# JuanJoZP/cfd-hemodynamic

Measured on AMD Instinct MI355X. Metric: time-steps/sec, dfg_1 ~1M DOF (stabilized_schur), higher is better.
Workload: dtype f64 (fp32 only in the AMG matrix values of the flexible preconditioner and in a read-only copy of the Krylov basis that Gram-Schmidt reads in solves of >= 20 iterations)

## Files before the change

cfd_hemodynamic_amd/_lib.py:

```python
from __future__ import annotations

import ctypes as C
import os
import subprocess

import numpy as np

_HERE = os.path.dirname(os.path.abspath(__file__))
_SO = os.path.join(_HERE, "libcfdh.so")
_LIB = None

dp = C.POINTER(C.c_double)
ip = C.POINTER(C.c_int32)
lp = C.POINTER(C.c_int64)


class Options(C.Structure):
    _fields_ = [
        ("snes_rtol", C.c_double), ("snes_atol", C.c_double), ("snes_stol", C.c_double), ("snes_max_it", C.c_int32),
        ("ksp_rtol", C.c_double), ("ksp_atol", C.c_double), ("ksp_max_it", C.c_int32), ("ksp_restart", C.c_int32),
        ("cheb_degree", C.c_int32), ("cheb_ratio", C.c_double), ("schur_full", C.c_int32),
        ("amg_smooth_degree", C.c_int32), ("amg_smooth_ratio", C.c_double), ("amg_theta", C.c_double),
        ("amg_max_coarse", C.c_int32), ("pc_refresh", C.c_int32), ("remove_p_mean", C.c_int32), ("verbose", C.c_int32),
        ("pc_type", C.c_int32), ("cc_smooth_degree", C.c_int32), ("ksp_guess", C.c_int32),
# ... 14 lines not shown
        ("ms_solve", C.c_double * 3), ("ms_total", C.c_double), ("launches", C.c_int32), ("host_syncs", C.c_int32),
    ]


ALLREDUCE_FN = C.CFUNCTYPE(C.c_int, C.c_void_p, dp, C.c_int, C.c_int)
EXCHANGE_FN = C.CFUNCTYPE(C.c_int, C.c_void_p, dp, dp)

SYMBOLS = [
    "cfdh_create", "cfdh_create_elem", "cfdh_create_elem_part", "cfdh_set_facet_markers", "cfdh_destroy", "cfdh_last_error", "cfdh_abi_version", "cfdh_set_params", "cfdh_default_options",
    "cfdh_set_options", "cfdh_clear_dirichlet", "cfdh_add_dirichlet", "cfdh_update_dirichlet", "cfdh_set_state", "cfdh_get_solution",
    "cfdh_get_previous", "cfdh_get_residual", "cfdh_advance", "cfdh_advance_field", "cfdh_set_time_scheme", "cfdh_set_previous2", "cfdh_get_previous2",
    "cfdh_shift_history", "cfdh_set_boundary_terms", "cfdh_set_formulation", "cfdh_set_pressure_boundaries", "cfdh_set_pressure_boundaries_ex", "cfdh_assemble", "cfdh_get_csr", "cfdh_spmv", "cfdh_solve_step",
    "cfdh_functional", "cfdh_wall_shear_stress", "cfdh_set_global_pressure_space", "cfdh_set_halo", "cfdh_comm_unique_id", "cfdh_comm_init", "cfdh_comm_set_callbacks",
    "cfdh_profile_enable", "cfdh_profile_get", "cfdh_profile_reset", "cfdh_info",
    "cfdh_set_schur_pcd", "cfdh_set_ksp_forcing", "cfdh_get_newton_history", "cfdh_get_pcd_operator", "cfdh_apply_preconditioner", "cfdh_apply_operator",
    "cfdh_get_amg_operator", "cfdh_get_amg_vectors", "cfdh_krylov_vec_op",
    "cfdh_create_ipcs", "cfdh_ipcs_set_form", "cfdh_ipcs_set_tolerances", "cfdh_ipcs_step", "cfdh_ipcs_get_operator", "cfdh_ipcs_get_intermediate",
    "cfdh_ipcs_apply_pressure_pc", "cfdh_ipcs_krylov_solve",
    "cfdh_wall_stats_reset", "cfdh_wall_stats_accumulate", "cfdh_wall_stats_get",
]


def build(force=False):
    src = os.path.join(_HERE, "csrc")
    newest = max(os.path.getmtime(os.path.join(src, f)) for f in os.listdir(src)
                 if f.endswith((".hip", ".cpp", ".hpp", ".h")))
    hdr = os.path.join(os.path.dirname(_HERE), "include", "cfdh.h")
    if os.path.exists(hdr):
        newest = max(newest, os.path.getmtime(hdr))
    if force or not os.path.exists(_SO) or os.path.getmtime(_SO) < newest:
# ... 51 lines not shown
    L.cfdh_set_global_pressure_space.argtypes = [vp, C.c_int64, C.c_int64, ip, dp, ip, C.c_int64, ip]
    L.cfdh_comm_unique_id.argtypes = [C.c_void_p]
    L.cfdh_comm_init.argtypes = [vp, C.c_void_p, C.c_int, C.c_int]
    L.cfdh_comm_set_callbacks.argtypes = [vp, ALLREDUCE_FN, EXCHANGE_FN, C.c_void_p, C.c_int, C.c_int]
    L.cfdh_profile_enable.argtypes = [vp, C.c_int]
    L.cfdh_profile_get.argtypes = [vp, C.c_int, dp, lp]
    L.cfdh_profile_reset.argtypes = [vp]
    L.cfdh_info.argtypes = [vp, C.c_int]
    L.cfdh_info.restype = C.c_int64
    L.cfdh_set_schur_pcd.argtypes = [vp, C.c_int, C.c_int, C.c_int]
    L.cfdh_set_ksp_forcing.argtypes = [vp, C.c_int, C.c_double, C.c_double, C.c_double, C.c_double, C.c_double]
    L.cfdh_get_newton_history.argtypes = [vp, ip, dp, dp, ip, dp]
    L.cfdh_get_pcd_operator.argtypes = [vp, lp, ip, ip, dp, dp]
    L.cfdh_apply_preconditioner.argtypes = [vp, dp, dp]
    L.cfdh_apply_operator.argtypes = [vp, dp, dp, dp]
    L.cfdh_get_amg_operator.argtypes = [vp, C.c_int, C.c_int, C.c_int, lp, lp, lp, ip, ip, dp]
    L.cfdh_get_amg_vectors.argtypes = [vp, C.c_int, C.c_int, C.c_int, lp, dp]
    L.cfdh_krylov_vec_op.argtypes = [vp, C.c_int, C.c_int, C.c_int, C.c_int, dp, dp, dp, dp, dp, C.c_double, C.c_int, dp, dp,
                                     C.POINTER(C.c_float), ip, dp, dp, dp]
    L.cfdh_create_ipcs.argtypes = [C.POINTER(vp), C.c_int, C.c_int, C.c_int64, C.c_int64, C.c_int64, ip, dp, C.c_int64, ip, ip, ip]
    L.cfdh_ipcs_set_form.argtypes = [vp, C.c_double, C.c_double]
    L.cfdh_ipcs_set_tolerances.argtypes = [vp, dp, C.c_double, ip]
    L.cfdh_ipcs_step.argtypes = [vp, C.POINTER(IpcsStats)]
    L.cfdh_ipcs_get_operator.argtypes = [vp, C.c_int, lp, ip, ip, dp]
    L.cfdh_ipcs_get_intermediate.argtypes = [vp, C.c_int, dp]
    L.cfdh_ipcs_apply_pressure_pc.argtypes = [vp, dp, dp]
    L.cfdh_ipcs_krylov_solve.argtypes = [vp, C.c_int, dp, dp, C.c_double, C.c_double, C.c_int, dp, C.POINTER(IpcsStats), dp]
    L.cfdh_wall_stats_reset.argtypes = [vp]
    L.cfdh_wall_stats_accumulate.argtypes = [vp, C.c_double]
    L.cfdh_wall_stats_get.argtypes = [vp, C.c_int, lp, dp]
# ... 318 lines not shown
        if r.size != (self.dim + 1) * self.nv:
            raise ValueError("monolithic vector of (gdim + 1) nv entries expected")
        z = np.zeros_like(r)
        self._chk(self.L.cfdh_apply_preconditioner(self.h, _dp(r), _dp(z)))
        return z

    def apply_operator(self, r):
        r = np.ascontiguousarray(r, dtype=np.float64)
        if r.size != (self.dim + 1) * self.nv:
            raise ValueError("monolithic vector of (gdim + 1) nv entries expected")
        z = np.zeros_like(r)
        w = np.zeros((self.dim + 1) * self.nvo)
        self._chk(self.L.cfdh_apply_operator(self.h, _dp(r), _dp(z), _dp(w)))
        return z, w

    def krylov_vec_op(self, op, n, ld, nvec=1, A=None, B=None, x=None, y=None, coef=None, scalar=0.0, flags=0):
        def arr(a, need, what):
            if a is None:
                return None
            a = np.ascontiguousarray(a, dtype=np.float64).ravel()
            if a.size < need:
                raise ValueError("%s: %d entries, %d needed" % (what, a.size, need))
            return a
        blk = max(n, 0) if op == KVOP_NORM2_TRIPLE else max(ld, 0) * max(nvec, 0)
        ncoef = {KVOP_GS_UPDATE_NORMALIZE: nvec + 1, KVOP_GUESS: 8 * (nvec + 1)}.get(op, nvec)
        A, B = arr(A, blk, "A"), arr(B, blk, "B")
        x, y, coef = arr(x, n, "x"), arr(y, n, "y"), arr(coef, ncoef, "coef")
        m = max(n, 1)
        out1, out2, out32 = np.zeros(m), np.zeros(m), np.zeros(m, dtype=np.float32)
        ns = max(nvec + 2, 72)
# ... 145 lines not shown
```

cfd_hemodynamic_amd/csrc/cfdh_api.cpp:

```cpp
#include <algorithm>
#include <cmath>
#include <numeric>

#include <dlfcn.h>

#include "cfdh_internal.hpp"
#include "cfdh_ipcs.hpp"

std::string g_cfdh_last_error;

int cfdh_prepare_assembly(cfdh_ctx *c);

#define ENTER(c)                         \
  do {                                   \
    if (!(c)) return CFDH_E_ARG;         \
    (void)hipSetDevice((c)->device);     \
  } while (0)

#define NOT_IPCS(c, name)                                                                                                    \
  do {                                                                                                                       \
    if ((c) && (c)->ipcs) return cfdh_fail((c), CFDH_E_STATE, name ": not available on an incremental pressure-correction context (cfdh_create_ipcs)"); \
  } while (0)
#define NEED_IPCS(c, name)                                                                                         \
  do {                                                                                                             \
// ... 63 lines not shown
  *out = nullptr;
  if (gdim != 2 && gdim != 3) return cfdh_fail(nullptr, CFDH_E_ARG, "gdim must be 2 (P1 triangles) or 3 (P1 tetrahedra)");
  if (etype < 0 || etype > 3) return cfdh_fail(nullptr, CFDH_E_ARG, "unknown element type %d", etype);
  if (!cells || !coords || (nfacets > 0 && (!facet_cells || !facet_local)))
    return cfdh_fail(nullptr, CFDH_E_ARG, "null mesh array");
  int ndev = 0;
  if (hipGetDeviceCount(&ndev) != hipSuccess || ndev <= 0)
    return cfdh_fail(nullptr, CFDH_E_HIP, "no HIP device available: libcfdh has no CPU fallback");
  if (device < 0 || device >= ndev) return cfdh_fail(nullptr, CFDH_E_ARG, "device %d out of range (%d devices)", device, ndev);
  cfdh_ctx *c = new (std::nothrow) cfdh_ctx();
  if (!c) return cfdh_fail(nullptr, CFDH_E_NOMEM, "out of host memory");
  c->device = device;
  cfdh_default_options(&c->opt);
  { const char *e = getenv("CFDH_NO_GRAPH"); c->use_graph = !(e && e[0] == '1'); }
  { const char *e = getenv("CFDH_SOLVE_LEAN"); c->lean = !(e && e[0] == '0'); }
  {
    cfdh_ctx::SolveEnv &v = c->env;
    const char *e;
    if ((e = getenv("CFDH_KRYLOV_FP32"))) v.krylov_fp32 = atoi(e);
    v.guess_check = getenv("CFDH_GUESS_CHECK") != nullptr;
    e = getenv("CFDH_NO_ATTAINABLE_STOP"); v.no_attainable_stop = e && e[0] == '1';
    if ((e = getenv("CFDH_GS_REFINE_FROM"))) v.gs_refine_from = atoi(e);
    if ((e = getenv("CFDH_KSP_LAG"))) v.ksp_lag = atoi(e);
    if ((e = getenv("CFDH_GS_ETA2"))) v.gs_eta2 = atof(e);
    if ((e = getenv("CFDH_L_CYCLES"))) v.l_cycles = atoi(e);
    if ((e = getenv("CFDH_A_CYCLES"))) v.a_cycles = atoi(e);
    e = getenv("CFDH_DL0_COARSE_SWEEPS"); v.dl0_coarse_sweeps = e && e[0] == '1';
  }
  if (c->use_graph && (getenv("ROCP_TOOL_LIBRARIES") || dlsym(RTLD_DEFAULT, "rocprofiler_configure"))) {
    int rt = 0;
// ... 550 lines not shown

int cfdh_apply_operator(cfdh_ctx *c, const double *r, double *z, double *w) {
  NOT_IPCS(c, "cfdh_apply_operator");
  if (!c || !r || !z || !w) return CFDH_E_ARG;
  ENTER(c);
  if (c->nranks > 1 || c->nvo != c->nv) return cfdh_fail(c, CFDH_E_STATE, "cfdh_apply_operator: one GPU only");
  if (!c->jac_valid) return cfdh_fail(c, CFDH_E_STATE, "no Jacobian assembled yet");
  CHK(cfdh_pc_update(c, false));
  std::vector<double> h;
  pack_vec(c, r, r + (size_t)c->dim * c->nv, h, nullptr);
  CHK(upload_vec(c, h, c->xt.p));
  CHK(cfdh_apply_operator_dev(c, c->xt.p, c->dvec.p));
  std::vector<double> oz, ow;
  CHK(download_vec(c, c->dvec.p, oz));
  CHK(download_vec(c, c->kw.p, ow));
  for (int k = 0; k < c->nvo; k++) {
    const int v = c->iperm[k], d = c->dim;
    for (int i = 0; i < d; i++) { z[(size_t)d * v + i] = oz[(size_t)d * k + i]; w[(size_t)d * v + i] = ow[(size_t)d * k + i]; }
    z[(size_t)d * c->nv + v] = oz[(size_t)d * c->nvo + k];
    w[(size_t)d * c->nvo + v] = ow[(size_t)d * c->nvo + k];
  }
  return 0;
}

int cfdh_krylov_vec_op(cfdh_ctx *c, int op, int n, int ld, int nvec, const double *A, const double *B, const double *x, const double *y,
                       const double *coef, double scalar, int flags, double *out1, double *out2, float *out32, int32_t *nscal,
                       double *scal_host, double *scal_dev, double *scal_mirror) {
  NOT_IPCS(c, "cfdh_krylov_vec_op");
  ENTER(c);
  if (c->nranks > 1 || c->nvo != c->nv) return cfdh_fail(c, CFDH_E_STATE, "cfdh_krylov_vec_op: one GPU only");
// ... 716 lines not shown
int cfdh_profile_get(cfdh_ctx *c, int kind, double *total_ms, int64_t *launches) {
  NOT_IPCS(c, "cfdh_profile_get");
  if (!c || kind < 0 || kind >= 12) return CFDH_E_ARG;
  prof_flush(c);
  if (total_ms) *total_ms = c->prof[kind].total_ms;
  if (launches) *launches = c->prof[kind].launches;
  return 0;
}
int cfdh_profile_reset(cfdh_ctx *c) {
  NOT_IPCS(c, "cfdh_profile_reset");
  ENTER(c);
  prof_flush(c);
  for (auto &p : c->prof) { p.total_ms = 0; p.launches = 0; }
  c->n_allreduce = c->n_halo = c->n_host_sync = c->n_krylov = c->n_allgather = 0;
  c->n_cycles = c->n_guess_projections = c->n_iter_sync = 0;
  c->n_krylov_discarded = 0;
  return 0;
}

int64_t cfdh_info(const cfdh_ctx *c, int what) {
  if (!c) return -1;
  if (c->ipcs) {
    const IpcsData *I = c->ipcs;
    switch (what) {
      case 0: case 1: return I->nn;
      case 2: return I->nc;
      case 3: return (int64_t)I->hM.col.size();
      case 6: return (int64_t)I->hLam.lev.size();
      case 15: return I->last.host_syncs;
      case 18: return 1;
// ... 38 lines not shown
      return ((what / 10) & 1) ? (int64_t)h.lev[l]->n : (int64_t)h.lev[l]->A.nnz;
    }
    case 28: return c->etype;
    case 70: return c->n_guess_solves;
    case 71: return c->n_guess_solves ? (int64_t)(1e6 * c->guess_reduction_sum / (double)c->n_guess_solves) : 0;
    case 29: return c->nloc;
    case 73: return c->n_krylov_discarded;
    case 74: return c->n_pc_builds;
    case 84: return c->n_cycles;
    case 86: return c->n_guess_projections;
    case 87: return c->n_iter_sync;
    case 88: return c->guess_last_rank;
    case 89: return c->guess_last_k;
    case 85: return c->lean ? 1 : 0;
    case 90: return c->ws_count;
    case 75: return c->pc_valid ? 1 : 0;
    case 76: return c->singular;
    case 77: return c->form;
    case 78: return c->opt.pc_type;
    case 79: return c->ew_version;
    case 72: return c->n_attainable_stops;
    case 27: return (int64_t)(1000.0 * c->ms_pc_build_dev);
    case 19: return c->opt.pc_type >= 1 ? c->hL.nnz_S0 : c->hS.nnz_S0;
    case 20: return c->hA.nnz_S0;
    case 21: return c->opt.pc_type >= 1 ? c->hL.nnz_G0 : c->hS.nnz_G0;
    case 22: return c->hA.nnz_G0;
    case 23: { const AmgHier &h = c->opt.pc_type >= 1 ? c->hL : c->hS; return h.lev.size() > 1 ? h.lev[1]->n : 0; }
    case 24: return c->hA.lev.size() > 1 ? c->hA.lev[1]->n : 0;
    case 25: { const AmgHier &h = c->opt.pc_type >= 1 ? c->hL : c->hS; return h.fused ? 1 : 0; }
    default: return -1;
// ... 121 lines not shown
```

cfd_hemodynamic_amd/csrc/cfdh_internal.hpp:

```cpp
#pragma once
#include <hip/hip_runtime.h>

#include <cstdint>
#include <cstdio>
#include <cstring>
#include <string>
#include <vector>

#include "cfdh.h"
#include "cfdh_scratch.hpp"

#ifndef CFDH_MAX_INC
#define CFDH_MAX_INC 256
#endif
#ifndef CFDH_MAX_BV
#define CFDH_MAX_BV 192
#endif
#ifndef CFDH_MAX_BC
#define CFDH_MAX_BC 192
#endif
#ifndef CFDH_MAX_ROWS
#define CFDH_MAX_ROWS 128
#endif

// ... 330 lines not shown
  int pcd_in = -1, pcd_out = -1, pcd_time = 0;
  double pcd_ct = 0;
  dbuf<int> pcd_iptr, pcd_inc, pcd_fptr, pcd_fac;
  dbuf<unsigned> pcd_islot, pcd_fslot;
  dbuf<int> pcd_sptr, pcd_scol, pcd_rlen;
  dbuf<double> pcd_K, pcd_mdinv, pcd_t, pcd_q;
  dbuf<float> pcd_Kf;
  dbuf<unsigned char> pcd_flag;
  std::vector<double> h_pcd_md;
  int ew_version = 0;
  double ew_rtol0 = 0.3, ew_rtol_max = 0.9, ew_gamma = 1.0, ew_alpha = 1.6180339887498949, ew_threshold = 0.1;
  std::vector<double> hist_fnorm, hist_rtol, hist_relres;
  std::vector<int> hist_its;
  double ksp_last_relres = 0;
  bool lean = true;
  struct SolveEnv {
    int krylov_fp32 = 1;
    bool guess_check = false;
    bool no_attainable_stop = false;
    int gs_refine_from = -1;
    int ksp_lag = KRING - 3;
    double gs_eta2 = 1e-6;
    int l_cycles = 1, a_cycles = 1;
    bool dl0_coarse_sweeps = false;
  } env;
  dbuf<double> qu;
  long long n_guess_projections = 0;
  int guess_last_rank = -1, guess_last_k = 0;
  long long n_iter_sync = 0;
  long long n_cycles = 0;
// ... 90 lines not shown
int k_halo_pack(cfdh_ctx *c, const double *vec);
int k_moments(cfdh_ctx *c);
int k_assemble(cfdh_ctx *c, const double *xstate, int mode);
int k_spmv_full(cfdh_ctx *c, const double *x, double *y);
int k_spmv_full_multi(cfdh_ctx *c, const double *X, double *Y, int ld, int nvec);
int k_spmv_block(cfdh_ctx *c, int blk, const double *x, double *y, const double *b, double alpha);
int k_spmv_block_ghost(cfdh_ctx *c, int blk, const double *xv, double *y, const double *b);
int k_extract_diag(cfdh_ctx *c);
int k_cheb_a00(cfdh_ctx *c, const double *b, double *x);
int k_cheb_a00_coeffs(cfdh_ctx *c);
int k_cheb_init(cfdh_ctx *c, int n, const double *dinv, const double *b, double *d0, double *x, double itheta, int accumulate,
                const double *coef);
int k_nullspace_test(cfdh_ctx *c, double *nrm, double *absnrm);
int k_spmv_a01_keep(cfdh_ctx *c, const double *x, double *y, const double *b, double *q);
int k_spmv_full_kept(cfdh_ctx *c, const double *x, double *y, const double *q);
int k_resid_norm(cfdh_ctx *c, const double *x, const double *b, double *r, double *nrm, bool *done);
int k_fnorm_nulltest(cfdh_ctx *c, int n, const double *F, double *fn, double *nrm, double *absnrm);
int k_bc_scatter(cfdh_ctx *c, int n, int ncomp, const int *idx, const unsigned char *flag, const double *val, const double *mult);
int v_pack_state(cfdh_ctx *c, const double *u_user, const double *p_user, double *dst);
int k_functional(cfdh_ctx *c, int kind, int marker, double *out);
int k_wss(cfdh_ctx *c, double *out);

int k_csr_spmv(cfdh_ctx *c, const CsrDev &A, const double *x, double *y, int mode, const double *b);
int k_csr_spmv_ncol(cfdh_ctx *c, const CsrDev &A, const double *x, double *y, int mode, const double *b, int ncol);
int k_amg_vcycle(cfdh_ctx *c, AmgHier &H, const double *b, double *x);
int k_level_smooth(cfdh_ctx *c, AmgLevel *L, const double *b, double *x, int degree);
bool k_cc_cheb2_scale(cfdh_ctx *c, AmgLevel *L, const double *b, double *x, const double *ml, double *y);
int k_cc_scale(cfdh_ctx *c, int n, const double *ml, const double *z, double *y);
int k_dl0_down(cfdh_ctx *c, const double *halo_vec);
int k_dl0_up(cfdh_ctx *c, double *out);
// ... 41 lines not shown
inline double *scalars_mirror(const cfdh_ctx *c) { return c->h_pinned_dev + HP_MIRROR; }
inline ScalarRead scalars_mirrored(int n) { return ScalarRead{nullptr, n, true}; }
int scalars_finish(cfdh_ctx *c, double *dev, int n, int op, int nblk, ScalarRead *h);
int scalars_read(cfdh_ctx *c, const ScalarRead &h, double *host, bool counted = true);

int comm_allreduce_dev(cfdh_ctx *c, double *dev, int n, int op);
int comm_allreduce_host(cfdh_ctx *c, double *v, int op);
int comm_allgather_dev(cfdh_ctx *c, const double *send, double *recv, int count);
int comm_halo(cfdh_ctx *c, double *vec);
int comm_finalize(cfdh_ctx *c);

int cfdh_pc_update(cfdh_ctx *c, bool force_refresh);
int cfdh_pc_apply(cfdh_ctx *c, const double *r, double *z);
int ensure_krylov(cfdh_ctx *c);
int cfdh_apply_operator_dev(cfdh_ctx *c, const double *r, double *z);
int cfdh_host_threads();
int cfdh_fgmres(cfdh_ctx *c, const double *b, double *x, int *its, int *reason, double bnorm = -1.0);
int v_norm2_pair(cfdh_ctx *c, int n, const double *x, const double *y, double *nx, double *ny);
int cfdh_newton_step(cfdh_ctx *c, cfdh_stats *st);
int cfdh_download_blocks(cfdh_ctx *c, std::vector<double> &a00, std::vector<double> &a01, std::vector<double> &a10,
                         std::vector<double> &a11);
```

cfd_hemodynamic_amd/csrc/cfdh_kernels.hip:

```cpp
#include <hip/hip_runtime.h>

#include <cmath>

#include "cfdh_internal.hpp"
#include "cfdh_quad_tri.h"
#include "cfdh_wave.hpp"

__constant__ double d_qw[CFDH_NQ];
__constant__ double d_ql[CFDH_NQ][3];

int k_upload_quadrature(cfdh_ctx *c) {
  HIPCHK(c, hipMemcpyToSymbol(HIP_SYMBOL(d_qw), CFDH_QW, sizeof(CFDH_QW)));
  HIPCHK(c, hipMemcpyToSymbol(HIP_SYMBOL(d_ql), CFDH_QL, sizeof(CFDH_QL)));
  return 0;
}

void prof_begin(cfdh_ctx *c, int kind) {
  if (!c->prof_on || c->capturing) return;
  if (c->ev_next + 2 > c->ev_pool.size()) {
    for (int i = 0; i < 64; i++) { hipEvent_t e; if (hipEventCreate(&e) != hipSuccess) return; c->ev_pool.push_back(e); }
  }
  cfdh_ctx::EvRec r;
  r.kind = kind; r.a = c->ev_pool[c->ev_next++]; r.b = c->ev_pool[c->ev_next++];
  (void)hipEventRecord(r.a, c->stream);
// ... 802 lines not shown
    if (KEPT) { const double2 qq = *(const double2 *)(q + 2 * (size_t)row); a0 += qq.x; a1 += qq.y; }
    if (RESID) {
      const double2 bu = *(const double2 *)(b + 2 * (size_t)row);
      a0 = bu.x - a0; a1 = bu.y - a1; a2 = b[2 * (size_t)nvo + row] - a2;
      ss = a0 * a0 + a1 * a1 + a2 * a2;
    }
    *(double2 *)(y + 2 * (size_t)row) = make_double2(a0, a1);
    y[2 * (size_t)nvo + row] = a2;
  }
  if (RESID) {
    ss = block_sum(ss, sh);
    if (threadIdx.x == 0) partial[blockIdx.x] = ss;
  }
}

int k_spmv_a01_keep(cfdh_ctx *c, const double *x, double *y, const double *b, double *q) {
  const long long n4 = 4ll * c->nvo;
  hipLaunchKernelGGL(spmv_a01_resid_kernel<true>, dim3((unsigned)((n4 + TPB - 1) / TPB)), dim3(TPB), 0, c->stream, c->nvo, c->vptr.p,
                     c->vcol.p, c->A01.p, x, y, b, q);
  HIPCHK(c, hipGetLastError());
  return 0;
}
int k_spmv_full_kept(cfdh_ctx *c, const double *x, double *y, const double *q) {
  const long long nthreads = 8ll * c->nvo;
  hipLaunchKernelGGL((spmv_full_lean_kernel<true, false>), dim3((unsigned)((nthreads + TPB - 1) / TPB)), dim3(TPB), 0, c->stream, c->nvo,
                     c->vptr.p, c->vcol.p, c->A00.p, c->A01.p, c->A10.p, c->A11.p, x, y, q, (const double *)nullptr, (double *)nullptr);
  HIPCHK(c, hipGetLastError());
  return 0;
}
int k_resid_norm(cfdh_ctx *c, const double *x, const double *b, double *r, double *nrm, bool *done) {
  const long long nthreads = 8ll * c->nvo;
  const long long nb = (nthreads + TPB - 1) / TPB;
  *done = false;
  if (c->dim != 2 || (size_t)nb > c->red_partial.n) return 0;
  hipLaunchKernelGGL((spmv_full_lean_kernel<false, true>), dim3((unsigned)nb), dim3(TPB), 0, c->stream, c->nvo, c->vptr.p, c->vcol.p, c->A00.p,
                     c->A01.p, c->A10.p, c->A11.p, x, r, (const double *)nullptr, b, c->red_partial.p);
  HIPCHK(c, hipGetLastError());
  CHK(red_final(c, 0, 1, (int)nb, (int)nb, c->red_partial.p, c->red_out.p + RO_LEAN_S2, scalars_mirror(c)));
  double s2;
  CHK(scalars_read(c, scalars_mirrored(1), &s2));
  *nrm = sqrt(s2);
// ... 403 lines not shown
```

cfd_hemodynamic_amd/csrc/cfdh_reduce.hip:

```cpp
#include <hip/hip_runtime.h>

#include "cfdh_internal.hpp"
#include "cfdh_wave.hpp"

#define TPB 256

int vgrid(int n) { int g = (n + TPB * 4 - 1) / (TPB * 4); return g < 1 ? 1 : (g > 2048 ? 2048 : g); }
int red_grid(const cfdh_ctx *c, int n) { const int g = vgrid(n); return g > c->red_blocks ? c->red_blocks : g; }

template <int OP>
__global__ __launch_bounds__(TPB) void reduce_partial_kernel(int n, const double *__restrict__ x, const double *__restrict__ y,
                                                             double *__restrict__ partial) {
  __shared__ double sh[4];
  double a = 0;
  for (int i = blockIdx.x * TPB + threadIdx.x; i < n; i += gridDim.x * TPB) {
    if (OP == 0) a += x[i] * y[i];
    else a = max_nan(a, fabs(y ? x[i] - y[i] : x[i]));
  }
  a = (OP == 0) ? block_sum(a, sh) : block_max(a, sh);
  if (threadIdx.x == 0) partial[blockIdx.x] = a;
}
template <int OP>
__global__ __launch_bounds__(TPB) void reduce_final_kernel(int nblk, int stride, const double *__restrict__ partial,
                                                           double *__restrict__ out, double *__restrict__ mirror = nullptr) {
  __shared__ double sh[4];
  const double *pp = partial + (size_t)blockIdx.x * stride;
  double a = 0;
  for (int i = threadIdx.x; i < nblk; i += TPB) a = (OP == 1) ? max_nan(a, pp[i]) : a + pp[i];
  a = (OP == 1) ? block_max(a, sh) : block_sum(a, sh);
  if (threadIdx.x == 0) {
    const double v = (OP == 2) ? sqrt(a) : a;
    out[blockIdx.x] = v;
    if (mirror) mirror[blockIdx.x] = v;
  }
}
__global__ __launch_bounds__(TPB) void mirror_copy_kernel(int n, const double *__restrict__ src, double *__restrict__ dst) {
  for (int i = threadIdx.x; i < n; i += TPB) dst[i] = src[i];
}
__global__ __launch_bounds__(TPB) void sum_partial_kernel(int n, const double *__restrict__ x, double *__restrict__ partial) {
  __shared__ double sh[4];
  double a = 0;
  for (int i = blockIdx.x * TPB + threadIdx.x; i < n; i += gridDim.x * TPB) a += x[i];
  a = block_sum(a, sh);
// ... 41 lines not shown
```

cfd_hemodynamic_amd/csrc/cfdh_solver.cpp:

```cpp
#include <algorithm>
#include <chrono>
#include <cmath>

#include "cfdh_internal.hpp"
#include "cfdh_krylov_host.hpp"

int cfdh_host_threads();

static double wall_ms() {
  using namespace std::chrono;
  return duration<double, std::milli>(steady_clock::now().time_since_epoch()).count();
}

int cfdh_download_blocks(cfdh_ctx *c, std::vector<double> &a00, std::vector<double> &a01, std::vector<double> &a10,
                         std::vector<double> &a11) {
  const size_t nz = (size_t)c->nnzv, d = (size_t)c->dim;
  a00.resize(d * d * nz); a01.resize(d * nz); a10.resize(d * nz); a11.resize(nz);
  HIPCHK(c, hipMemcpyAsync(a00.data(), c->A00.p, sizeof(double) * d * d * nz, hipMemcpyDeviceToHost, c->stream));
  HIPCHK(c, hipMemcpyAsync(a01.data(), c->A01.p, sizeof(double) * d * nz, hipMemcpyDeviceToHost, c->stream));
  HIPCHK(c, hipMemcpyAsync(a10.data(), c->A10.p, sizeof(double) * d * nz, hipMemcpyDeviceToHost, c->stream));
  HIPCHK(c, hipMemcpyAsync(a11.data(), c->A11.p, sizeof(double) * nz, hipMemcpyDeviceToHost, c->stream));
  HIPCHK(c, hipStreamSynchronize(c->stream));
  return 0;
}
// ... 695 lines not shown
    } else {
      for (int st = 0; st < 6; st++) { HIPCHK(c, hipGraphLaunch(pg->exec[st], c->stream)); CHK(pc_exchange(c, st)); }
    }
  }
  if (c->singular) CHK(v_sub_mean(c, nvo, z + (size_t)c->dim * nvo));
  return 0;
}

static int pc_then_product(cfdh_ctx *c, const double *r, double *z, double *w) {
  CHK(cfdh_pc_apply(c, r, z));
  CHK(comm_halo(c, z));
  if (lean_keep_qu(c) && !c->prof_on) return k_spmv_full_kept(c, z, w, c->qu.p);
  return k_spmv_full(c, z, w);
}

static size_t krylov_ld(const cfdh_ctx *c) { return ((size_t)c->NL + 1) & ~(size_t)1; }

int cfdh_apply_operator_dev(cfdh_ctx *c, const double *r, double *z) {
  CHK(ensure_krylov(c));
  return pc_then_product(c, r, z, c->kw.p);
}

int ensure_krylov(cfdh_ctx *c) {
  const int m = c->opt.ksp_restart;
  if (c->kry_m == m && c->kV.p) return 0;
  const size_t NL = krylov_ld(c);
  c->pc_graph_valid = false;
  HIPCHK(c, c->kV.alloc(NL * (m + 1)));
  HIPCHK(c, c->kZ.alloc(NL * m));
  HIPCHK(c, c->kw.alloc(NL));
  HIPCHK(c, c->kh.alloc(std::max(2 * (size_t)(m + 2) + 8, (size_t)8 * (8 + 1))));
  HIPCHK(c, c->ky.alloc(m + 8));
  if (c->h_ring) { (void)hipHostFree(c->h_ring); c->h_ring = nullptr; }
  c->h_ring_stride = ((size_t)m + 5) & ~(size_t)1;
  HIPCHK(c, hipHostMalloc((void **)&c->h_ring, sizeof(double) * c->h_ring_stride * (cfdh_ctx::KRING + 1)));
  HIPCHK(c, hipHostGetDevicePointer((void **)&c->h_ring_dev, c->h_ring, 0));
  for (auto &e : c->ev_ring) if (!e) HIPCHK(c, hipEventCreateWithFlags(&e, hipEventDisableTiming));
  HIPCHK(c, c->kV.zero(c->stream)); HIPCHK(c, c->kZ.zero(c->stream)); HIPCHK(c, c->kw.zero(c->stream));
  if ((size_t)(m + 2) * 1024 > c->red_partial.n) HIPCHK(c, c->red_partial.alloc((size_t)(m + 2) * 1024 + 1024));
  c->kry_m = m;
  return 0;
}

static int guess_ensure(cfdh_ctx *c) {
  const int m = c->opt.ksp_guess;
  const size_t ld = krylov_ld(c);
  if (m == c->guess_m && (m == 0 || c->guessU.p)) return 0;
  c->guess_m = m;
  for (int k = 0; k < cfdh_ctx::GUESS_NEWTON; k++) c->guess_cnt[k] = c->guess_head[k] = 0;
  if (m > 0) {
    HIPCHK(c, c->guessU.alloc(ld * (size_t)m * cfdh_ctx::GUESS_NEWTON)); HIPCHK(c, c->guessU.zero(c->stream));
    HIPCHK(c, c->guessX.alloc(ld * (size_t)cfdh_ctx::GUESS_NEWTON));
  }
  return 0;
// ... 247 lines not shown
    s.last_true = beta;
  } else {
    s.last_true = -1.0;
  }
  s.beta_start = beta;
  return 0;
}

static int fgmres_launch(Fgmres &s, int jj) {
  cfdh_ctx *c = s.c;
  const int n = s.n, m = s.m;
  const size_t ld = s.ld, ld32 = s.ld32;
  double *V = c->kV.p, *w = c->kw.p, *hd = c->kh.p, *s_dev = hd + 2 * (m + 2) + 1;
  double *vj = V + (size_t)jj * ld, *zj = c->kZ.p + (size_t)jj * ld, *vn = V + (size_t)(jj + 1) * ld;
  double *slot = c->h_ring_dev + (size_t)(jj % cfdh_ctx::KRING) * c->h_ring_stride;
  CHK(pc_then_product(c, vj, zj, w));
  if (s.use32) {
    CHK(v_multidot32(c, n, s.V32, (int)ld32, jj + 1, w, hd, slot));
    CHK(v_gs_update32(c, n, s.V32, (int)ld32, jj + 1, hd, w, vn, s.V32 + (size_t)(jj + 1) * ld32, s_dev, slot + (jj + 2)));
    HIPCHK(c, hipEventRecord(c->ev_ring[jj % cfdh_ctx::KRING], c->stream));
  } else {
    CHK(v_multidot(c, n, V, (int)ld, jj + 1, w, hd, true, slot));
    HIPCHK(c, hipEventRecord(c->ev_ring[jj % cfdh_ctx::KRING], c->stream));
    CHK(v_gs_update_normalize(c, n, V, (int)ld, jj + 1, hd, w, vn, s_dev));
  }
  return 0;
}

static int fgmres_second_pass(Fgmres &s, int j, const double *hs, double ww, double hh2, double *hnorm) {
  cfdh_ctx *c = s.c;
  const int n = s.n, m = s.m;
  double *V = c->kV.p, *hd = c->kh.p, *vn = V + (size_t)(j + 1) * s.ld;
  CHK(v_multidot(c, n, V, (int)s.ld, j + 1, vn, hd + (m + 2), true));
  CHK(v_multiaxpy(c, n, V, (int)s.ld, j + 1, hd + (m + 2), vn));
  if (s.use32) CHK(v_norm_to_dev(c, n, vn, hd + 2 * (m + 2)));
  double *h2 = s.hh.data() + Fgmres::HH2_AT(m);
  CHK(scalars_read(c, ScalarRead{hd + (m + 2), m + 4, false}, h2));
// ... 295 lines not shown
```

include/cfdh.h:

```cpp
#ifndef CFDH_H
#define CFDH_H

#include <stdint.h>

#ifdef __cplusplus
extern "C" {
#endif

#define CFDH_ABI_VERSION 1

enum {
  CFDH_OK = 0,
  CFDH_E_ARG = -1,
  CFDH_E_HIP = -2,
  CFDH_E_STATE = -3,
  CFDH_E_DIVERGED = -4,
  CFDH_E_COMM = -5,
  CFDH_E_NOMEM = -6
};

enum {
  CFDH_CONVERGED_FNORM_ABS = 2,
  CFDH_CONVERGED_FNORM_RELATIVE = 3,
  CFDH_CONVERGED_SNORM_RELATIVE = 4,
// ... 77 lines not shown


enum { CFDH_FORM_CONVECTIVE = 0, CFDH_FORM_ROTATIONAL = 1 };
int cfdh_set_formulation(cfdh_ctx *ctx, int form);
int cfdh_set_pressure_boundaries(cfdh_ctx *ctx, int n, const int32_t *markers, const double *values, double beta_nitsche);
int cfdh_set_pressure_boundaries_ex(cfdh_ctx *ctx, int n, const int32_t *markers, const double *values, double beta_nitsche,
                                    const uint8_t *nitsche, const double *beta_backflow);


int cfdh_set_schur_pcd(cfdh_ctx *ctx, int inlet_marker, int outlet_marker, int time_term);
int cfdh_set_ksp_forcing(cfdh_ctx *ctx, int version, double rtol_0, double rtol_max, double gamma, double alpha, double threshold);
int cfdh_get_newton_history(cfdh_ctx *ctx, int32_t *n, double *fnorm, double *ksp_rtol, int32_t *ksp_its, double *ksp_rel_res);
int cfdh_get_pcd_operator(cfdh_ctx *ctx, int64_t *nnz, int32_t *rowptr, int32_t *col, double *vals, double *mass_diag);
int cfdh_apply_preconditioner(cfdh_ctx *ctx, const double *r, double *z);
int cfdh_apply_operator(cfdh_ctx *ctx, const double *r, double *z, double *w);

#define CFDH_AMG_HIER_A 0
#define CFDH_AMG_HIER_P 1
#define CFDH_AMG_HIER_H 2
#define CFDH_AMG_HIER_PG 3
#define CFDH_AMG_HIER_DL0 4
#define CFDH_AMG_OP_A 0
#define CFDH_AMG_OP_P 1
#define CFDH_AMG_OP_G 2
#define CFDH_AMG_OP_SB 3
#define CFDH_AMG_OP_SC 4
#define CFDH_AMG_OP_PT 5
int cfdh_get_amg_operator(cfdh_ctx *ctx, int hier, int level, int which, int64_t *nrow, int64_t *ncol, int64_t *nnz, int32_t *rowptr,
                          int32_t *col, double *vals);
#define CFDH_AMG_VEC_DINV 0
// ... 106 lines not shown
```

Baseline: 443.5.

## Fuse Krylov basis dot products into the kept-q operator SpMV kernel

Adds a kernel that computes the full lean SpMV product and, in the same pass, the dot products of the result against the existing Krylov basis vectors plus its own squared norm. It writes per-block partials that red_final reduces. In fp64 FGMRES iterations this replaces the separate multidot pass, so w is not re-read from memory. The final-reduction loop is also unrolled eightfold to load more partials in flight. The cost is extra registers and basis loads inside the SpMV kernel, a cap of 31 basis vectors, and support for 2D only.

```diff
diff --git a/cfd_hemodynamic_amd/_lib.py b/cfd_hemodynamic_amd/_lib.py
--- a/cfd_hemodynamic_amd/_lib.py
+++ b/cfd_hemodynamic_amd/_lib.py
@@ -52,6 +52,7 @@
     "cfdh_functional", "cfdh_wall_shear_stress", "cfdh_set_global_pressure_space", "cfdh_set_halo", "cfdh_comm_unique_id", "cfdh_comm_init", "cfdh_comm_set_callbacks",
     "cfdh_profile_enable", "cfdh_profile_get", "cfdh_profile_reset", "cfdh_info",
     "cfdh_set_schur_pcd", "cfdh_set_ksp_forcing", "cfdh_get_newton_history", "cfdh_get_pcd_operator", "cfdh_apply_preconditioner", "cfdh_apply_operator",
+    "cfdh_apply_operator_dots",
     "cfdh_get_amg_operator", "cfdh_get_amg_vectors", "cfdh_krylov_vec_op",
     "cfdh_create_ipcs", "cfdh_ipcs_set_form", "cfdh_ipcs_set_tolerances", "cfdh_ipcs_step", "cfdh_ipcs_get_operator", "cfdh_ipcs_get_intermediate",
     "cfdh_ipcs_apply_pressure_pc", "cfdh_ipcs_krylov_solve",
@@ -133,6 +134,7 @@
     L.cfdh_get_pcd_operator.argtypes = [vp, lp, ip, ip, dp, dp]
     L.cfdh_apply_preconditioner.argtypes = [vp, dp, dp]
     L.cfdh_apply_operator.argtypes = [vp, dp, dp, dp]
+    L.cfdh_apply_operator_dots.argtypes = [vp, dp, C.c_int, C.c_int, dp, dp, dp, dp, ip]
     L.cfdh_get_amg_operator.argtypes = [vp, C.c_int, C.c_int, C.c_int, lp, lp, lp, ip, ip, dp]
     L.cfdh_get_amg_vectors.argtypes = [vp, C.c_int, C.c_int, C.c_int, lp, dp]
     L.cfdh_krylov_vec_op.argtypes = [vp, C.c_int, C.c_int, C.c_int, C.c_int, dp, dp, dp, dp, dp, C.c_double, C.c_int, dp, dp,
@@ -481,6 +483,18 @@
         self._chk(self.L.cfdh_apply_operator(self.h, _dp(r), _dp(z), _dp(w)))
         return z, w
 
+    def apply_operator_dots(self, r, V):
+        r = np.ascontiguousarray(r, dtype=np.float64)
+        V = np.ascontiguousarray(V, dtype=np.float64)
+        if r.size != (self.dim + 1) * self.nv or V.ndim != 2 or V.shape[1] < r.size:
+            raise ValueError("monolithic vector of (gdim + 1) nv entries and a block of rows at least that long expected")
+        z = np.zeros_like(r)
+        w = np.zeros((self.dim + 1) * self.nvo)
+        h = np.zeros(V.shape[0] + 1)
+        fused = np.zeros(1, dtype=np.int32)
+        self._chk(self.L.cfdh_apply_operator_dots(self.h, _dp(r), V.shape[0], V.shape[1], _dp(V), _dp(z), _dp(w), _dp(h), _ip(fused)))
+        return z, w, h, int(fused[0])
+
     def krylov_vec_op(self, op, n, ld, nvec=1, A=None, B=None, x=None, y=None, coef=None, scalar=0.0, flags=0):
         def arr(a, need, what):
             if a is None:
diff --git a/cfd_hemodynamic_amd/csrc/cfdh_api.cpp b/cfd_hemodynamic_amd/csrc/cfdh_api.cpp
--- a/cfd_hemodynamic_amd/csrc/cfdh_api.cpp
+++ b/cfd_hemodynamic_amd/csrc/cfdh_api.cpp
@@ -101,6 +101,7 @@
   cfdh_default_options(&c->opt);
   { const char *e = getenv("CFDH_NO_GRAPH"); c->use_graph = !(e && e[0] == '1'); }
   { const char *e = getenv("CFDH_SOLVE_LEAN"); c->lean = !(e && e[0] == '0'); }
+  { const char *e = getenv("CFDH_FUSED_DOTS"); c->fused_dots = !(e && e[0] == '0'); }
   {
     cfdh_ctx::SolveEnv &v = c->env;
     const char *e;
@@ -681,6 +682,46 @@
   std::vector<double> oz, ow;
   CHK(download_vec(c, c->dvec.p, oz));
   CHK(download_vec(c, c->kw.p, ow));
+  for (int k = 0; k < c->nvo; k++) {
+    const int v = c->iperm[k], d = c->dim;
+    for (int i = 0; i < d; i++) { z[(size_t)d * v + i] = oz[(size_t)d * k + i]; w[(size_t)d * v + i] = ow[(size_t)d * k + i]; }
+    z[(size_t)d * c->nv + v] = oz[(size_t)d * c->nvo + k];
+    w[(size_t)d * c->nvo + v] = ow[(size_t)d * c->nvo + k];
+  }
+  return 0;
+}
+
+int cfdh_apply_operator_dots(cfdh_ctx *c, const double *r, int nvec, int ld, const double *V, double *z, double *w, double *h, int32_t *fused) {
+  NOT_IPCS(c, "cfdh_apply_operator_dots");
+  if (!c || !r || !V || !z || !w || !h || !fused) return CFDH_E_ARG;
+  ENTER(c);
+  if (c->nranks > 1 || c->nvo != c->nv) return cfdh_fail(c, CFDH_E_STATE, "cfdh_apply_operator_dots: one GPU only");
+  if (!c->jac_valid) return cfdh_fail(c, CFDH_E_STATE, "no Jacobian assembled yet");
+  const size_t nmono = (size_t)(c->dim + 1) * c->nv;
+  if (nvec < 1 || (size_t)nvec + 2 > (size_t)HP_MIRROR_N) return cfdh_fail(c, CFDH_E_ARG, "cfdh_apply_operator_dots: nvec = %d outside 1 .. %d", nvec, (int)HP_MIRROR_N - 2);
+  if (ld < 0 || (size_t)ld < nmono) return cfdh_fail(c, CFDH_E_ARG, "cfdh_apply_operator_dots: ld = %d below the vector length %zu", ld, nmono);
+  CHK(cfdh_pc_update(c, false));
+  const size_t kld = ((size_t)c->NL + 1) & ~(size_t)1;
+  std::vector<double> hv, blk(kld * (size_t)nvec, 0.0);
+  for (int v = 0; v < nvec; v++) {
+    const double *col = V + (size_t)v * (size_t)ld;
+    pack_vec(c, col, col + (size_t)c->dim * c->nv, hv, nullptr);
+    std::copy(hv.begin(), hv.end(), blk.begin() + (size_t)v * kld);
+  }
+  HookBuf<double> dV, dh;
+  CHK(dV.put(c, blk.data(), blk.size(), blk.size()));
+  CHK(dh.put(c, nullptr, (size_t)nvec + 2, 0));
+  pack_vec(c, r, r + (size_t)c->dim * c->nv, hv, nullptr);
+  CHK(upload_vec(c, hv, c->xt.p));
+  bool f = false;
+  CHK(cfdh_apply_operator_dots_dev(c, c->xt.p, c->dvec.p, dV.p, kld, nvec, dh.p, scalars_mirror(c), &f));
+  *fused = f ? 1 : 0;
+  std::vector<double> oz, ow;
+  CHK(download_vec(c, c->dvec.p, oz));
+  CHK(download_vec(c, c->kw.p, ow));
+  CHK(dh.get(c, h, (size_t)nvec + 1));
+  const double *mir = c->h_pinned + HP_MIRROR;
+  if (memcmp(mir, h, sizeof(double) * ((size_t)nvec + 1)) != 0) return cfdh_fail(c, CFDH_E_STATE, "cfdh_apply_operator_dots: the host-mapped copy of h differs from the device's");
   for (int k = 0; k < c->nvo; k++) {
     const int v = c->iperm[k], d = c->dim;
     for (int i = 0; i < d; i++) { z[(size_t)d * v + i] = oz[(size_t)d * k + i]; w[(size_t)d * v + i] = ow[(size_t)d * k + i]; }
@@ -1427,6 +1468,7 @@
   for (auto &p : c->prof) { p.total_ms = 0; p.launches = 0; }
   c->n_allreduce = c->n_halo = c->n_host_sync = c->n_krylov = c->n_allgather = 0;
   c->n_cycles = c->n_guess_projections = c->n_iter_sync = 0;
+  c->n_fused_iters = 0;
   c->n_krylov_discarded = 0;
   return 0;
 }
@@ -1495,6 +1537,7 @@
     case 89: return c->guess_last_k;
     case 85: return c->lean ? 1 : 0;
     case 90: return c->ws_count;
+    case 91: return c->n_fused_iters;
     case 75: return c->pc_valid ? 1 : 0;
     case 76: return c->singular;
     case 77: return c->form;
diff --git a/cfd_hemodynamic_amd/csrc/cfdh_internal.hpp b/cfd_hemodynamic_amd/csrc/cfdh_internal.hpp
--- a/cfd_hemodynamic_amd/csrc/cfdh_internal.hpp
+++ b/cfd_hemodynamic_amd/csrc/cfdh_internal.hpp
@@ -368,6 +368,8 @@
   std::vector<int> hist_its;
   double ksp_last_relres = 0;
   bool lean = true;
+  bool fused_dots = true;
+  long long n_fused_iters = 0;
   struct SolveEnv {
     int krylov_fp32 = 1;
     bool guess_check = false;
@@ -488,6 +490,9 @@
 int k_nullspace_test(cfdh_ctx *c, double *nrm, double *absnrm);
 int k_spmv_a01_keep(cfdh_ctx *c, const double *x, double *y, const double *b, double *q);
 int k_spmv_full_kept(cfdh_ctx *c, const double *x, double *y, const double *q);
+int k_spmv_full_kept_dots_blocks(const cfdh_ctx *c, int nvec);
+size_t k_spmv_full_kept_dots_workspace(const cfdh_ctx *c, int max_nout);
+int k_spmv_full_kept_dots(cfdh_ctx *c, const double *x, double *y, const double *q, const double *V, size_t ld, int nvec);
 int k_resid_norm(cfdh_ctx *c, const double *x, const double *b, double *r, double *nrm, bool *done);
 int k_fnorm_nulltest(cfdh_ctx *c, int n, const double *F, double *fn, double *nrm, double *absnrm);
 int k_bc_scatter(cfdh_ctx *c, int n, int ncomp, const int *idx, const unsigned char *flag, const double *val, const double *mult);
@@ -559,6 +564,7 @@
 int cfdh_pc_apply(cfdh_ctx *c, const double *r, double *z);
 int ensure_krylov(cfdh_ctx *c);
 int cfdh_apply_operator_dev(cfdh_ctx *c, const double *r, double *z);
+int cfdh_apply_operator_dots_dev(cfdh_ctx *c, const double *r, double *z, const double *V, size_t ld, int nvec, double *h_dev, double *mirror, bool *fused);
 int cfdh_host_threads();
 int cfdh_fgmres(cfdh_ctx *c, const double *b, double *x, int *its, int *reason, double bnorm = -1.0);
 int v_norm2_pair(cfdh_ctx *c, int n, const double *x, const double *y, double *nx, double *ny);
diff --git a/cfd_hemodynamic_amd/csrc/cfdh_kernels.hip b/cfd_hemodynamic_amd/csrc/cfdh_kernels.hip
--- a/cfd_hemodynamic_amd/csrc/cfdh_kernels.hip
+++ b/cfd_hemodynamic_amd/csrc/cfdh_kernels.hip
@@ -840,6 +840,83 @@
   }
 }
 
+#define FD_ROWS (TPB / 8)
+template <int NT>
+__global__ __launch_bounds__(TPB) void spmv_full_kept_dots_kernel(int nvo, const int *__restrict__ vptr, const int *__restrict__ vcol,
+                                                                  const double *__restrict__ A00, const double *__restrict__ A10,
+                                                                  const double *__restrict__ A11, const double *__restrict__ x,
+                                                                  double *__restrict__ y, const double *__restrict__ q,
+                                                                  const double *__restrict__ V, size_t ld, int nvec,
+                                                                  double *__restrict__ partial) {
+  static_assert(NT >= 1 && NT <= 4, "8 NT values per block, at most 32");
+  __shared__ double sh[4 * 8 * NT];
+  const int l = threadIdx.x & 7;
+  constexpr int NPRE = NT <= 2 ? NT : 2;
+  double d[NT];
+  {
+    const int row = blockIdx.x * FD_ROWS + (threadIdx.x >> 3);
+    double2 vxy[NT];
+    double vp[NT];
+    const size_t lo = (size_t)l * ld;
+    auto load_basis = [&](int t) {
+      const int v = l + 8 * t;
+      vxy[t] = make_double2(0.0, 0.0); vp[t] = 0.0;
+      if (row < nvo && v < nvec) {
+        const double *Vv = V + (size_t)(8 * t) * ld;
+        vxy[t] = *(const double2 *)(Vv + (lo + 2 * (size_t)row));
+        vp[t] = Vv[lo + 2 * (size_t)nvo + row];
+      }
+    };
+#pragma unroll
+    for (int t = 0; t < NPRE; t++) load_basis(t);
+    double a0 = 0, a1 = 0, a2 = 0;
+    if (row < nvo) {
+      const int ks = vptr[row], ke = vptr[row + 1];
+      for (int k = ks + l; k < ke; k += 8) {
+        const int w = vcol[k];
+        const int uo = uoff(w, nvo), po = poff(w, nvo);
+        const double xu0 = x[uo], xu1 = x[uo + 1], xp = x[po];
+        const double2 b0 = *(const double2 *)(A00 + 4 * (size_t)k), b1 = *(const double2 *)(A00 + 4 * (size_t)k + 2);
+        const double2 c10 = *(const double2 *)(A10 + 2 * (size_t)k);
+        const double c11 = A11[k];
+        a0 += b0.x * xu0 + b0.y * xu1;
+        a1 += b1.x * xu0 + b1.y * xu1;
+        a2 += c10.x * xu0 + c10.y * xu1 + c11 * xp;
+      }
+    }
+#pragma unroll
+    for (int t = NPRE; t < NT; t++) load_basis(t);
+    a0 = group8_sum(a0); a1 = group8_sum(a1); a2 = group8_sum(a2);
+    if (row < nvo) {
+      const double2 qq = *(const double2 *)(q + 2 * (size_t)row);
+      a0 += qq.x; a1 += qq.y;
+      if (l == 0) {
+        *(double2 *)(y + 2 * (size_t)row) = make_double2(a0, a1);
+        y[2 * (size_t)nvo + row] = a2;
+      }
+    }
+#pragma unroll
+    for (int t = 0; t < NT; t++) {
+      const int v = l + 8 * t;
+      d[t] = v < nvec ? a0 * vxy[t].x + a1 * vxy[t].y + a2 * vp[t] : (v == nvec ? a0 * a0 + a1 * a1 + a2 * a2 : 0.0);
+    }
+  }
+  const int lane = threadIdx.x & 63, wv = threadIdx.x >> 6;
+#pragma unroll
+  for (int t = 0; t < NT; t++) {
+    double s = d[t];
+    s += dpp_shuffle<0x128>(s);
+    s += __shfl_xor(s, 16);
+    s += __shfl_xor(s, 32);
+    if (lane < 8) sh[wv * 8 * NT + l + 8 * t] = s;
+  }
+  __syncthreads();
+  if ((int)threadIdx.x < 8 * NT && (int)threadIdx.x <= nvec) {
+    const int v = threadIdx.x;
+    partial[(size_t)v * gridDim.x + blockIdx.x] = (sh[v] + sh[8 * NT + v]) + (sh[2 * 8 * NT + v] + sh[3 * 8 * NT + v]);
+  }
+}
+
 int k_spmv_a01_keep(cfdh_ctx *c, const double *x, double *y, const double *b, double *q) {
   const long long n4 = 4ll * c->nvo;
   hipLaunchKernelGGL(spmv_a01_resid_kernel<true>, dim3((unsigned)((n4 + TPB - 1) / TPB)), dim3(TPB), 0, c->stream, c->nvo, c->vptr.p,
@@ -851,6 +928,31 @@
   const long long nthreads = 8ll * c->nvo;
   hipLaunchKernelGGL((spmv_full_lean_kernel<true, false>), dim3((unsigned)((nthreads + TPB - 1) / TPB)), dim3(TPB), 0, c->stream, c->nvo,
                      c->vptr.p, c->vcol.p, c->A00.p, c->A01.p, c->A10.p, c->A11.p, x, y, q, (const double *)nullptr, (double *)nullptr);
+  HIPCHK(c, hipGetLastError());
+  return 0;
+}
+int k_spmv_full_kept_dots_blocks(const cfdh_ctx *c, int nvec) {
+  const int nout = nvec + 1;
+  const long long nb = ((long long)c->nvo + FD_ROWS - 1) / FD_ROWS;
+  if (c->dim != 2 || nvec < 1 || nout > 32 || nb < 1 || (size_t)nout * (size_t)nb > c->red_partial.n) return 0;
+  return (int)nb;
+}
+size_t k_spmv_full_kept_dots_workspace(const cfdh_ctx *c, int max_nout) {
+  return (size_t)std::min(max_nout, 32) * (((size_t)c->nvo + FD_ROWS - 1) / FD_ROWS);
+}
+int k_spmv_full_kept_dots(cfdh_ctx *c, const double *x, double *y, const double *q, const double *V, size_t ld, int nvec) {
+  const int nb = k_spmv_full_kept_dots_blocks(c, nvec);
+  if (nb == 0) return cfdh_fail(c, CFDH_E_STATE, "product with %d fused dot products: beyond the kernel's limits", nvec);
+#define LAUNCH_DOTS(NT)                                                                                                              \
+  hipLaunchKernelGGL((spmv_full_kept_dots_kernel<NT>), dim3((unsigned)nb), dim3(TPB), 0, c->stream, c->nvo, c->vptr.p, c->vcol.p, c->A00.p, \
+                     c->A10.p, c->A11.p, x, y, q, V, ld, nvec, c->red_partial.p)
+  switch ((nvec + 1 + 7) / 8) {
+    case 1: LAUNCH_DOTS(1); break;
+    case 2: LAUNCH_DOTS(2); break;
+    case 3: LAUNCH_DOTS(3); break;
+    default: LAUNCH_DOTS(4); break;
+  }
+#undef LAUNCH_DOTS
   HIPCHK(c, hipGetLastError());
   return 0;
 }
diff --git a/cfd_hemodynamic_amd/csrc/cfdh_reduce.hip b/cfd_hemodynamic_amd/csrc/cfdh_reduce.hip
--- a/cfd_hemodynamic_amd/csrc/cfdh_reduce.hip
+++ b/cfd_hemodynamic_amd/csrc/cfdh_reduce.hip
@@ -26,7 +26,15 @@
   __shared__ double sh[4];
   const double *pp = partial + (size_t)blockIdx.x * stride;
   double a = 0;
-  for (int i = threadIdx.x; i < nblk; i += TPB) a = (OP == 1) ? max_nan(a, pp[i]) : a + pp[i];
+  int i = threadIdx.x;
+  for (; i + 7 * TPB < nblk; i += 8 * TPB) {
+    double p[8];
+#pragma unroll
+    for (int u = 0; u < 8; u++) p[u] = pp[i + u * TPB];
+#pragma unroll
+    for (int u = 0; u < 8; u++) a = (OP == 1) ? max_nan(a, p[u]) : a + p[u];
+  }
+  for (; i < nblk; i += TPB) a = (OP == 1) ? max_nan(a, pp[i]) : a + pp[i];
   a = (OP == 1) ? block_max(a, sh) : block_sum(a, sh);
   if (threadIdx.x == 0) {
     const double v = (OP == 2) ? sqrt(a) : a;
diff --git a/cfd_hemodynamic_amd/csrc/cfdh_solver.cpp b/cfd_hemodynamic_amd/csrc/cfdh_solver.cpp
--- a/cfd_hemodynamic_amd/csrc/cfdh_solver.cpp
+++ b/cfd_hemodynamic_amd/csrc/cfdh_solver.cpp
@@ -733,11 +733,34 @@
   return k_spmv_full(c, z, w);
 }
 
+static bool fused_dots_apply(const cfdh_ctx *c, int nvec) {
+  return c->fused_dots && lean_keep_qu(c) && !c->prof_on && k_spmv_full_kept_dots_blocks(c, nvec) > 0;
+}
+static int pc_product_dots(cfdh_ctx *c, const double *r, double *z, double *w, int n, const double *V, size_t ld, int nvec, double *h_dev,
+                           double *mirror, bool *fused) {
+  *fused = fused_dots_apply(c, nvec);
+  if (!*fused) {
+    CHK(pc_then_product(c, r, z, w));
+    return v_multidot(c, n, V, (int)ld, nvec, w, h_dev, true, mirror);
+  }
+  CHK(cfdh_pc_apply(c, r, z));
+  CHK(comm_halo(c, z));
+  CHK(k_spmv_full_kept_dots(c, z, w, c->qu.p, V, ld, nvec));
+  const int nb = k_spmv_full_kept_dots_blocks(c, nvec);
+  return red_final(c, 0, nvec + 1, nb, nb, c->red_partial.p, h_dev, mirror);
+}
+
 static size_t krylov_ld(const cfdh_ctx *c) { return ((size_t)c->NL + 1) & ~(size_t)1; }
 
 int cfdh_apply_operator_dev(cfdh_ctx *c, const double *r, double *z) {
   CHK(ensure_krylov(c));
   return pc_then_product(c, r, z, c->kw.p);
+}
+int cfdh_apply_operator_dots_dev(cfdh_ctx *c, const double *r, double *z, const double *V, size_t ld, int nvec, double *h_dev, double *mirror,
+                                 bool *fused) {
+  CHK(ensure_krylov(c));
+  if ((size_t)(nvec + 2) * 1024 > c->red_partial.n) HIPCHK(c, c->red_partial.alloc((size_t)(nvec + 2) * 1024 + 1024));
+  return pc_product_dots(c, r, z, c->kw.p, c->NO, V, ld, nvec, h_dev, mirror, fused);
 }
 
 int ensure_krylov(cfdh_ctx *c) {
@@ -756,7 +779,9 @@
   HIPCHK(c, hipHostGetDevicePointer((void **)&c->h_ring_dev, c->h_ring, 0));
   for (auto &e : c->ev_ring) if (!e) HIPCHK(c, hipEventCreateWithFlags(&e, hipEventDisableTiming));
   HIPCHK(c, c->kV.zero(c->stream)); HIPCHK(c, c->kZ.zero(c->stream)); HIPCHK(c, c->kw.zero(c->stream));
-  if ((size_t)(m + 2) * 1024 > c->red_partial.n) HIPCHK(c, c->red_partial.alloc((size_t)(m + 2) * 1024 + 1024));
+  size_t need = (size_t)(m + 2) * 1024;
+  if (c->fused_dots && c->dim == 2) need = std::max(need, k_spmv_full_kept_dots_workspace(c, m + 2));
+  if (need > c->red_partial.n) HIPCHK(c, c->red_partial.alloc(need + 1024));
   c->kry_m = m;
   return 0;
 }
@@ -1034,13 +1059,15 @@
   double *V = c->kV.p, *w = c->kw.p, *hd = c->kh.p, *s_dev = hd + 2 * (m + 2) + 1;
   double *vj = V + (size_t)jj * ld, *zj = c->kZ.p + (size_t)jj * ld, *vn = V + (size_t)(jj + 1) * ld;
   double *slot = c->h_ring_dev + (size_t)(jj % cfdh_ctx::KRING) * c->h_ring_stride;
-  CHK(pc_then_product(c, vj, zj, w));
   if (s.use32) {
+    CHK(pc_then_product(c, vj, zj, w));
     CHK(v_multidot32(c, n, s.V32, (int)ld32, jj + 1, w, hd, slot));
     CHK(v_gs_update32(c, n, s.V32, (int)ld32, jj + 1, hd, w, vn, s.V32 + (size_t)(jj + 1) * ld32, s_dev, slot + (jj + 2)));
     HIPCHK(c, hipEventRecord(c->ev_ring[jj % cfdh_ctx::KRING], c->stream));
   } else {
-    CHK(v_multidot(c, n, V, (int)ld, jj + 1, w, hd, true, slot));
+    bool fused = false;
+    CHK(pc_product_dots(c, vj, zj, w, n, V, ld, jj + 1, hd, slot, &fused));
+    if (fused) c->n_fused_iters++;
     HIPCHK(c, hipEventRecord(c->ev_ring[jj % cfdh_ctx::KRING], c->stream));
     CHK(v_gs_update_normalize(c, n, V, (int)ld, jj + 1, hd, w, vn, s_dev));
   }
diff --git a/include/cfdh.h b/include/cfdh.h
--- a/include/cfdh.h
+++ b/include/cfdh.h
@@ -115,6 +115,7 @@
 int cfdh_get_pcd_operator(cfdh_ctx *ctx, int64_t *nnz, int32_t *rowptr, int32_t *col, double *vals, double *mass_diag);
 int cfdh_apply_preconditioner(cfdh_ctx *ctx, const double *r, double *z);
 int cfdh_apply_operator(cfdh_ctx *ctx, const double *r, double *z, double *w);
+int cfdh_apply_operator_dots(cfdh_ctx *ctx, const double *r, int nvec, int ld, const double *V, double *z, double *w, double *h, int32_t *fused);
 
 #define CFDH_AMG_HIER_A 0
 #define CFDH_AMG_HIER_P 1
```

Result: faster. 450.9 (median of 5 runs) (+1.7%).
